# Eurus-Holmes/VAG-NMT

Hardware: AMD Instinct MI355X
Metric: training sentence-pairs/sec (Multi30K en->de, B=64) (higher is better)
Workload: dtype f32; 1 GPU; configs[1]: multimodal en->de train step, B=64/GPU, Ts=Tt=40, E=256, H=512, S=512, I=2048, Vs=8507, V=9391, dropout 0.3/0.5/0.5, tied emb, teacher_force_ratio=1; global_batch=64, parallelism=dp1, hip_graph=True

## Files before the change

### vag-nmt_amd/csrc/api.hip

```cpp
#include "../../include/vag_nmt.h"
#include "kernels.h"
#include <cstring>

#define S_(x) reinterpret_cast<hipStream_t>(x)

static inline int zero_async(void* p, size_t bytes, hipStream_t s) {
    if (bytes == 0) return VAG_OK;
    return vag_axpy_launch(0.f, reinterpret_cast<const float*>(p), reinterpret_cast<float*>(p), (int64_t)(bytes / 4), 2, s);
}
static inline int copy_async(void* dst, const void* src, size_t bytes, hipStream_t s) {
    if (bytes == 0) return VAG_OK;
    return vag_axpy_launch(1.f, reinterpret_cast<const float*>(src), reinterpret_cast<float*>(dst), (int64_t)(bytes / 4), 0, s);
}
static int linear_fwd(int64_t M, int64_t N, int64_t K, const float* x, int64_t ldx, const float* W, const float* bias,
                      int act, float* y, int64_t ldy, hipStream_t s) {
    if (M <= 256) return vag_skinny_launch(M, N, K, x, ldx, W, K, bias, nullptr, 0, y, ldy, act, s);
    return vag_gemm_launch(M, N, K, 1.f, x, ldx, 1, W, 1, K, 0.f, y, ldy, bias, act, s);
}
static int gemm_tn_acc(int64_t M, int64_t N, int64_t R, const float* A, int64_t lda, const float* B, int64_t ldb, float* C,
                       int64_t ldc, hipStream_t s, float* g_bias = nullptr) {
    if (R == 0) return VAG_OK;
    return vag_gemm_launch(M, N, R, 1.f, A, 1, lda, B, ldb, 1, 1.f, C, ldc, nullptr, VAG_ACT_NONE, s, 0, g_bias);
}
static int gemm_nn(int64_t M, int64_t N, int64_t K, const float* A, int64_t lda, const float* B, int64_t ldb, float beta,
// ... 31 lines not shown
}

static void* head_dl16_slot(float* logits, int64_t ldl, int64_t R, int64_t CH, int64_t E) {
    if (!head_grads_one_plane() || CH <= 128 || vag_opt().head_bf16_dlogits == 0) return nullptr;
    if (E <= 64 || vag_opt().gemm_f32mfma != 0 || vag_opt().gemm_force_tile != 0) return nullptr;
    if (CH * 3 > R * 2) return nullptr;
    return logits + CH * ldl;
}

VagOptions& vag_opt() {
    static VagOptions o;
    return o;
}

extern "C" {

int vag_version(void) { return 330; }

int vag_set_option(const char* name, int64_t value) {
    VAG_CHECK_ARG(name != nullptr);
    VagOptions& o = vag_opt();
    const struct { const char* n; int* p; } ints[] = {
        {"gemm_f32mfma", &o.gemm_f32mfma}, {"gemm_slabs", &o.gemm_slabs}, {"gemm_nogroup", &o.gemm_nogroup}, {"gemm_big", &o.gemm_big}, {"gemm_force_tile", &o.gemm_force_tile},
        {"gemm_force_splitk", &o.gemm_force_splitk}, {"head_fuse", &o.head_fuse},
        {"head_bf16_grads", &o.head_bf16_grads}, {"persistent", &o.persistent}, {"persistent_dec_bwd", &o.persistent_dec_bwd}, {"persistent_enc_bwd", &o.persistent_enc_bwd}, {"free_persistent", &o.free_persistent}, {"attn_dot_reg", &o.attn_dot_reg},
        {"persist_timing", &o.persist_timing}, {"s16_one_plane", &o.s16_one_plane}, {"leaf_queue", &o.leaf_queue}, {"attn_row", &o.attn_row}, {"dec_xcd_map", &o.dec_xcd_map}, {"loss_ride", &o.loss_ride}, {"step_fork", &o.step_fork},
        {"head_bf16_dlogits", &o.head_bf16_dlogits}};
    for (const auto& e : ints)
        if (strcmp(name, e.n) == 0) { *e.p = (int)value; return VAG_OK; }
    if (strcmp(name, "head_chunk") == 0) { o.head_chunk = value; return VAG_OK; }
    if (strcmp(name, "persist_spin_limit") == 0) { o.persist_spin_limit = value; return VAG_OK; }
#ifdef VAG_LAB
    if (strcmp(name, "dec_stamps") == 0) { o.dec_stamps = value; return VAG_OK; }
    if (strcmp(name, "dec_bwd_stamps") == 0) { o.dec_bwd_stamps = value; return VAG_OK; }
    if (strcmp(name, "gemm_debug") == 0) { o.gemm_debug = (int)value; return VAG_OK; }
    if (strcmp(name, "gemm_planes") == 0) {
        g_base_ctx.gemm_planes = (value == 2 || value == 1 || value == 11) ? (int)value : 3;
        return VAG_OK;
    }
#endif
    return VAG_EINVAL;
}

int vag_set_operator_context(const float* derived, int storage) {
    VAG_CHECK_ARG(storage == 0 || (storage == 1 && derived));
    g_base_ctx.derived = derived;
    g_base_ctx.store16 = storage == 1;
// ... 945 lines not shown
    const int64_t R = Tt * B;
    if (!inv_cnt_ready) VAG_TRY(vag_inv_cnt_launch(tgt, B, Tt, inv_cnt, s));
    VagCallCtx::HeadFuse& hf = vag_ctx().head_fuse;
    const int64_t hc = vag_ctx().head_chunk;
    const int64_t CH = (!logits_ready && hc > 0 && hc < R) ? (hc + B - 1) / B * B : 0;
    if (CH > 0) {
        VAG_TRY(head_pre_seq(h2_all, c_all, e_all, w, R, E, H, p_out, rng, tmid, s));
        for (int64_t r0 = 0; r0 < R; r0 += CH) {
            const int64_t rows = R - r0 < CH ? R - r0 : CH;
            VAG_TRY(vag_gemm_launch(rows, V, E, 1.f, tmid + r0 * E, E, 1, w.out_w, 1, E, 0.f, logits, ldl, w.out_b, 0, s));
            VAG_TRY(vag_lse_nll_launch(logits, ldl, rows, V, tgt + r0 / B, B, Tt, vocab_weight, lse + r0, nll + r0, nullptr, 0,
                                       nullptr, 0, s, eps));
            if (hf.g) {
                const vag_head_g& g = *hf.g;
                void* dl16 = rows > 128 ? head_dl16_slot(logits, ldl, R, CH, E) : nullptr;
                VAG_TRY(vag_ce_bwd_colsum_launch(logits, ldl, rows, V, tgt + r0 / B, B, Tt, vocab_weight, lse + r0, inv_cnt,
                                                 hf.d_loss, g.out_b, s, dl16, eps));
                VAG_TRY(head_dt_gemm(rows, E, V, logits, ldl, w.out_w, hf.dt + r0 * E, s, dl16));
                VAG_TRY(head_outw_gemm(V, E, rows, logits, ldl, tmid + r0 * E, g.out_w, s, dl16));
            }
        }
        if (hf.g) hf.done = true;
    } else {
        if (!logits_ready) {
            VAG_TRY(head_pre_seq(h2_all, c_all, e_all, w, R, E, H, p_out, rng, tmid, s));
            VAG_TRY(vag_gemm_launch(R, V, E, 1.f, tmid, E, 1, w.out_w, 1, E, 0.f, logits, ldl, w.out_b, 0, s));
        }
        VAG_TRY(vag_lse_nll_launch(logits, ldl, R, V, tgt, B, Tt, vocab_weight, lse, nll, nullptr, 0, nullptr, 0, s, eps));
    }
    if (losses) return vag_loss_mt_mix_launch(nll, inv_cnt, B, Tt, losses, w_mt, w_vse, has_vse, s);
    return vag_loss_mt_launch(nll, inv_cnt, B, Tt, loss_mt, s);
}
extern "C" {

static int head_bwd_data(const vag_head_w& w, int64_t R, int64_t E, int64_t H, int64_t V, float p_out, const uint64_t* rng,
                         const float* tmid, const float* dlogits, int64_t ldl, float* d_h2_all, float* d_c_all,
                         float* d_e_all, float* dt, hipStream_t s, bool dt_ready = false) {
    const int64_t C = 2 * H;
    if (!dt_ready) VAG_TRY(head_dt_gemm(R, E, V, dlogits, ldl, w.out_w, dt, s));
    VAG_TRY(vag_tanh_bwd_launch(tmid, dt, dt, R * E, rng, VAG_DROP_DEC_OUT, p_out, s));
    VagGemmGroup grp5;
    VAG_TRY(gemm_nn(R, H, E, dt, E, w.w1, H, 0.f, d_h2_all, H, s));
    VAG_TRY(gemm_nn(R, C, E, dt, E, w.w2, C, 0.f, d_c_all, C, s));
    VAG_TRY(gemm_nn(R, E, E, dt, E, w.w3, E, 0.f, d_e_all, E, s));
    return grp5.end(s);
}
static int head_bwd_weights(const float* h2_all, const float* c_all, const float* e_all, int64_t R, int64_t E, int64_t H,
                            int64_t V, const float* tmid, const float* dlogits, int64_t ldl, const float* dt,
                            const vag_head_g& g, hipStream_t s, bool out_b_done = false, bool out_w_done = false) {
    const int64_t C = 2 * H;
    VagGemmGroup grp6;
// ... 548 lines not shown
```

### vag-nmt_amd/csrc/call_ctx.h

```cpp
#pragma once
#include <hip/hip_runtime.h>
#include <stdint.h>
#include "../../include/vag_nmt.h"

struct LossTask {
    const float* nll = nullptr; const float* inv_cnt = nullptr; float* losses = nullptr;
    int B = 0, Tt = 0, has_vse = 0, ring = 0;
    float w_mt = 0.f, w_vse = 0.f;
};
struct RmwDefer {
    float* out = nullptr;
    const float *a1 = nullptr, *x1 = nullptr, *a2 = nullptr, *x2 = nullptr;
    const float *mask = nullptr, *dx = nullptr; float coef = 0.f;
    int64_t B = 0, Ts = 0, C = 0;
};

struct VagCallCtx {
    const float* derived = nullptr;
    bool store16 = false;
    int gemm_planes = 3;
    unsigned* guard = nullptr;

    int64_t head_chunk = 0;
    struct HeadFuse { const vag_head_g* g = nullptr; const float* d_loss = nullptr; float* dt = nullptr; bool done = false; } head_fuse;
    bool step_zeroed = false;
    bool step_gathered = false;
    bool poison_inject = false;
    bool persist_prezeroed = false;
    int loss_ring = 0;
    struct GemmScratch { float* slab = nullptr; int64_t floats = 0; unsigned* tickets = nullptr; int64_t ntickets = 0; hipStream_t stream = nullptr; } gemm_scratch;
    const float* gemm_prezeroed[4] = {nullptr, nullptr, nullptr, nullptr};
    struct LeafStream { hipStream_t stream = nullptr; hipEvent_t event = nullptr; bool used = false; } leaf_stream;

    struct RowMix { float* xmix = nullptr; float split = 0.f; const float* done = nullptr; } row_mix;
    struct Dh0Tanh { bool req = false; const float* done = nullptr; } dh0_tanh;
    struct LossDefer { bool on = false; LossTask task; hipStream_t stream = nullptr; } loss_defer;
    RmwDefer rmw;
    bool leaf_on = false;
    const float* u_all_ready = nullptr;
};

VagCallCtx& vag_ctx();

struct VagCallScope {
    VagCallCtx& ctx;
    VagCallCtx* prev;
    explicit VagCallScope(VagCallCtx& c);
    ~VagCallScope();
    VagCallScope(const VagCallScope&) = delete;
    VagCallScope& operator=(const VagCallScope&) = delete;
};
```

### vag-nmt_amd/csrc/common.h

```cpp
#pragma once
#include <hip/hip_runtime.h>
#include <stdint.h>
#include <stddef.h>

#define VAG_OK 0
#define VAG_EINVAL (-22)
#define VAG_ENOSYS (-38)

#define VAG_CHECK_ARG(cond)                     \
    do {                                        \
        if (!(cond)) return VAG_EINVAL;         \
    } while (0)

#define VAG_LAUNCH_CHECK()                                  \
    do {                                                    \
        hipError_t e__ = hipGetLastError();                 \
        if (e__ != hipSuccess) return (int)e__;             \
    } while (0)

#define VAG_TRY(expr)                  \
    do {                               \
        int r__ = (expr);              \
        if (r__ != 0) return r__;      \
    } while (0)
// ... 51 lines not shown
__device__ __forceinline__ float h16_hi(unsigned p) { return (float)__builtin_bit_cast(vag_half, (unsigned short)(p >> 16)); }
template <bool XH> __device__ __forceinline__ float4 ld4_any(const float* base, int64_t elem) {
    if (XH) {
        const uint2 p = *reinterpret_cast<const uint2*>(reinterpret_cast<const vag_half*>(base) + elem);
        return make_float4(h16_lo(p.x), h16_hi(p.x), h16_lo(p.y), h16_hi(p.y));
    }
    return *reinterpret_cast<const float4*>(base + elem);
}
template <bool XH> __device__ __forceinline__ float ld1_any(const float* base, int64_t elem) {
    if (XH) return (float)reinterpret_cast<const vag_half*>(base)[elem];
    return base[elem];
}

struct VagOptions {
    int gemm_f32mfma = 0;
    int gemm_big = 1;
    int gemm_slabs = 1;
    int gemm_nogroup = 0;
    int gemm_force_tile = 0;
    int gemm_force_splitk = 0;
    int gemm_debug = 0;
    int64_t head_chunk = -1;
    int head_fuse = 1;
    int head_bf16_grads = 1;
    int persistent = 1;
    int persistent_dec_bwd = 1;
    int persistent_enc_bwd = 1;
    int attn_dot_reg = 1;
    int free_persistent = 1;
    int s16_one_plane = 1;
    int head_bf16_dlogits = 1;
    int leaf_queue = 1;
    int attn_row = 1;
    int loss_ride = 1;
    int dec_xcd_map = 33;
    int step_fork = 0;
    int64_t persist_spin_limit = 0;
    int persist_timing = 0;
    int64_t dec_bwd_stamps = 0;
    int64_t dec_stamps = 0;
};
VagOptions& vag_opt();

enum { VAG_ACT_NONE = 0, VAG_ACT_TANH = 1 };
enum { VAG_DROP_ENC_EMB = 1, VAG_DROP_ENC_CTX = 2, VAG_DROP_DEC_OUT = 3 };

// ... 94 lines not shown
```

### vag-nmt_amd/csrc/gemm.hip

```cpp
#ifndef VAG_CHEAT_B
#define VAG_CHEAT_B 0
#endif
#include "gemm_shared.h"
#include "call_ctx.h"
#include <algorithm>
#include <atomic>
#include <cstdio>
#include <cstdlib>
#include <functional>
int vag_copy2d_launch(const float* in, int64_t ldi, float* out, int64_t ldo, int64_t rows, int64_t cols, hipStream_t s);

template <int BT, bool KC, bool VEC, int NTH>
__device__ __forceinline__ void tile_load(const float* __restrict__ P, int64_t so, int64_t sk, int o0, int k0,
                                          int OUT, int KEND, float4 (&r)[BT * (BK / 4) / NTH]) {
    const int tid = threadIdx.x;
#pragma unroll
    for (int i = 0; i < BT * (BK / 4) / NTH; ++i) {
        const int idx = tid + i * NTH;
        float4 v = make_float4(0.f, 0.f, 0.f, 0.f);
        if (KC) {
            const int o = o0 + idx / (BK / 4), k = k0 + ((idx % (BK / 4)) << 2);
            if (o < OUT) {
                const float* p = P + (int64_t)o * so + k;
                if (VEC && k + 3 < KEND) {
// ... 131 lines not shown
    int tiles_x[LEAF_MAX];
    int n;
};
__global__ __launch_bounds__(256) void gemm_tiled_multi_kernel(LeafTasks T) {
    __shared__ __attribute__((aligned(16))) float smem[2 * BK * 68 + 2 * BK * 68];
    int k = 0;
    while (k + 1 < T.n && (int)blockIdx.x >= T.tile0[k + 1]) ++k;
    const int t = blockIdx.x - T.tile0[k];
    const GemmArgs& a = T.g[k];
    const int bx = t % T.tiles_x[k], by = t / T.tiles_x[k];
    if (a.rowsum && bx == 0 && threadIdx.x < 64) {
        const int m = by * 64 + threadIdx.x;
        if (m < a.M) {
            float s0 = 0.f, s1 = 0.f;
            int r = 0;
            for (; r + 1 < a.K; r += 2) { s0 += a.A[(int64_t)r * a.sa_k + m]; s1 += a.A[(int64_t)(r + 1) * a.sa_k + m]; }
            if (r < a.K) s0 += a.A[(int64_t)r * a.sa_k + m];
            a.rowsum[m] += s0 + s1;
        }
    }
    gemm_tiled_body<64, 64, false, false, true, 256>(a, smem, bx, by, 0);
}

template <bool AKC, bool BKC, bool VEC, int PL = 3, bool F16 = false, bool ABF = false>
__device__ __forceinline__ void gemm_split_body(const GemmArgs& a, __bf16* smem, int bx, int by, int bz) {
    __bf16* As = smem;
    __bf16* Bs = smem + PL * SP_PLANE;
    const int m0 = by * 128, n0 = bx * 128;
    const int kbeg = bz * a.kchunk;
    const int kend = min(a.K, kbeg + a.kchunk);
    const int lane = threadIdx.x & 63, wave = threadIdx.x >> 6;
    const int wm = wave >> 2, wn = wave & 3;

    f32x16 acc[2];
#pragma unroll
    for (int i = 0; i < 2; ++i)
#pragma unroll
        for (int r = 0; r < 16; ++r) acc[i][r] = 0.f;

    const __bf16* Af = As + (wm * 64 + (lane & 31)) * SP_LD + 8 * (lane >> 5);
    const __bf16* Bf = Bs + (wn * 32 + (lane & 31)) * SP_LD + 8 * (lane >> 5);

    SpRegs ra, rb;
    constexpr bool FAST = VEC && !ABF;
    const int nt = (kend - kbeg + SP_BK - 1) / SP_BK;
    const int nfull = FAST ? (kend - kbeg) / SP_BK : 0;
    SpFast<AKC> fa;
// ... 75 lines not shown
            for (int r = 0; r < 16; ++r) acc[i][r] = 0.f;
        const float4* all = reinterpret_cast<const float4*>(a.slab) + (int64_t)tile * a.nslices * 4096 + (wave * 8) * 64 + lane;
        for (int z = 0; z < a.nslices; ++z) {
            f32x4 v[8];
            const float4* p = all + (int64_t)z * 4096;
            asm volatile("global_load_dwordx4 %0, %8, off sc1\n\tglobal_load_dwordx4 %1, %8, off offset:1024 sc1\n\t"
                         "global_load_dwordx4 %2, %8, off offset:2048 sc1\n\tglobal_load_dwordx4 %3, %8, off offset:3072 sc1\n\t"
                         "global_load_dwordx4 %4, %9, off sc1\n\tglobal_load_dwordx4 %5, %9, off offset:1024 sc1\n\t"
                         "global_load_dwordx4 %6, %9, off offset:2048 sc1\n\tglobal_load_dwordx4 %7, %9, off offset:3072 sc1\n\t"
                         "s_waitcnt vmcnt(0)"
                         : "=&v"(v[0]), "=&v"(v[1]), "=&v"(v[2]), "=&v"(v[3]), "=&v"(v[4]), "=&v"(v[5]), "=&v"(v[6]), "=&v"(v[7])
                         : "v"(p), "v"(p + 256) : "memory");
#pragma unroll
            for (int i = 0; i < 2; ++i)
#pragma unroll
                for (int q = 0; q < 4; ++q)
#pragma unroll
                    for (int e = 0; e < 4; ++e) acc[i][4 * q + e] += v[i * 4 + q][e];
        }
        atomic = a.beta != 0.f;
        first = true;
    }
    const int col = n0 + wn * 32 + (lane & 31);
    if (col >= a.N) return;
    const float bv = (a.bias && first) ? a.bias[col] : 0.f;
#pragma unroll
    for (int i = 0; i < 2; ++i) {
        const int row0 = m0 + wm * 64 + i * 32 + 4 * (lane >> 5);
        if (a.c_half) gemm_epilogue16(acc[i], a.C, a.ldc, a.M - row0, a.alpha, a.beta, bv, a.act, atomic, 1, (int64_t)row0 * a.ldc + col);
        else gemm_epilogue16(acc[i], a.C + (int64_t)row0 * a.ldc + col, a.ldc, a.M - row0, a.alpha, a.beta, bv, a.act, atomic);
    }
}

template <bool AKC, bool BKC, bool VEC, int PL = 3, bool F16 = false, bool ABF = false>
__global__ __launch_bounds__(512, PL == 1 ? 6 : 4) void gemm_split_kernel(GemmArgs a) {
    __shared__ __attribute__((aligned(16))) __bf16 smem[2 * PL * SP_PLANE];
    gemm_split_body<AKC, BKC, VEC, PL, F16, ABF>(a, smem, blockIdx.x, blockIdx.y, blockIdx.z);
}

template <bool AKC, bool BKC, int PL = 3, bool F16 = false>
__global__ __launch_bounds__(512, PL == 1 ? 6 : 4) void gemm_split_group_kernel(GemmGroupArgs G) {
    __shared__ __attribute__((aligned(16))) __bf16 smem[2 * PL * SP_PLANE];
    int p = 0;
    while (p + 1 < G.n && (int)blockIdx.x >= G.start[p + 1]) ++p;
    const GemmArgs& a = G.p[p];
    const int id = blockIdx.x - G.start[p];
    const int tn = (a.N + 127) / 128, tm = (a.M + 127) / 128;
    const int bx = id % tn, by = (id / tn) % tm, bz = id / (tn * tm);
    gemm_split_body<AKC, BKC, true, PL, F16>(a, smem, bx, by, bz);
}

constexpr int BIG_STAGE = 4 * SP_PLANE;
constexpr int BIG_LDS_BYTES = 2 * BIG_STAGE * 2;
__device__ __forceinline__ void big_barrier() { asm volatile("s_waitcnt lgkmcnt(0)\n\ts_barrier" ::: "memory"); }

template <bool AKC, bool BKC, bool F16, bool ABF>
__device__ __forceinline__ void gemm_big_body(const GemmArgs& a, __bf16* smem, int bx, int by, int bz) {
    const int m0 = by * 256, n0 = bx * 256;
    const int kbeg = bz * a.kchunk;
    const int kend = min(a.K, kbeg + a.kchunk);
// ... 138 lines not shown
    const GemmArgs& a = G.p[p];
    const int id = blockIdx.x - G.start[p];
    const int tn = (a.N + 255) / 256, tm = (a.M + 255) / 256;
    const int bx = id % tn, by = (id / tn) % tm, bz = id / (tn * tm);
    gemm_big_body<AKC, BKC, F16, false>(a, big_smem, bx, by, bz);
}
template <typename K> static bool big_attr(K kernel) {
    static std::atomic<unsigned long long> done{0};
    int dev = 0;
    if (hipGetDevice(&dev) != hipSuccess || dev < 0 || dev >= 64) return false;
    if (done.load(std::memory_order_acquire) & (1ull << dev)) return true;
    if (hipFuncSetAttribute(reinterpret_cast<const void*>(kernel), hipFuncAttributeMaxDynamicSharedMemorySize, BIG_LDS_BYTES) != hipSuccess)
        return false;
    done.fetch_or(1ull << dev, std::memory_order_release);
    return true;
}

static int gemm_split_dispatch(const GemmArgs& g, bool akc, bool bkc, bool vec, dim3 grid, hipStream_t s) {
    const int gemm_planes = vag_ctx().gemm_planes;
    if (g.a_bf16) {
        if (gemm_planes != 1 || bkc || !vec) return VAG_EINVAL;
        if (akc) hipLaunchKernelGGL((gemm_split_kernel<true, false, true, 1, false, true>), grid, dim3(512), 0, s, g);
        else hipLaunchKernelGGL((gemm_split_kernel<false, false, true, 1, false, true>), grid, dim3(512), 0, s, g);
        VAG_LAUNCH_CHECK();
        return VAG_OK;
    }
#define VAG_SPLIT_CASE(AK, BKc, V)                                                                    \
    if (akc == AK && bkc == BKc && vec == V) {                                                        \
        if (gemm_planes == 2) hipLaunchKernelGGL((gemm_split_kernel<AK, BKc, V, 2>), grid, dim3(512), 0, s, g);   \
        else if (gemm_planes == 1) hipLaunchKernelGGL((gemm_split_kernel<AK, BKc, V, 1>), grid, dim3(512), 0, s, g);   \
        else if (gemm_planes == 11) hipLaunchKernelGGL((gemm_split_kernel<AK, BKc, V, 1, true>), grid, dim3(512), 0, s, g);   \
        else hipLaunchKernelGGL((gemm_split_kernel<AK, BKc, V, 3>), grid, dim3(512), 0, s, g);        \
        VAG_LAUNCH_CHECK();                                                                           \
        return VAG_OK;                                                                                \
    }
    VAG_SPLIT_CASE(true, true, true)
    VAG_SPLIT_CASE(true, false, true)
    VAG_SPLIT_CASE(false, true, true)
    VAG_SPLIT_CASE(false, false, true)
    VAG_SPLIT_CASE(true, true, false)
    VAG_SPLIT_CASE(true, false, false)
    VAG_SPLIT_CASE(false, true, false)
    VAG_SPLIT_CASE(false, false, false)
#undef VAG_SPLIT_CASE
    return VAG_EINVAL;
}
// ... 347 lines not shown
            if (sp > 1 && (!can_split || K / sp < 128)) break;
            const int64_t kper = cdiv64(cdiv64(K, sp), BK) * BK;
            const int64_t blocks = base * sp;
            double rounds;
            if (t == 128 && !opt_f32mfma) {
                const int64_t full = blocks / 512, rem = blocks % 512;
                rounds = 1.5 * (double)full + (rem == 0 ? 0.0 : (rem <= 256 ? 1.0 : 1.5));
            } else {
                rounds = (double)cdiv64(blocks, 256);
            }
            const double t_mfma = rounds * (double)kper * (double)(t * t) * 2.0 / (256.0 * eff) / 2400.0;
            const double bytes = (double)M * (double)N * 4.0;
            const bool slabs_on = gemm_slabs_usable(stream) && t == 128 && gemm_planes == 3 && !opt_f32mfma;
            const double t_out = sp > 1 ? (slabs_on ? sp * bytes / 4.0e6 + 1.5 * sp + bytes / (beta != 0.f ? atomic_rate : 4.0e6)
                                                    : sp * bytes / atomic_rate + (beta == 0.f ? bytes / 4.0e6 + 2.0 : 0.0))
                                        : bytes * (beta != 0.f ? 2.0 : 1.0) / 4.0e6;
            const double cost = t_mfma + t_out;
            if (cost < best) { best = cost; T = t; splitk = sp; }
        }
    }
    {
        const int ft = vag_opt().gemm_force_tile, fs = vag_opt().gemm_force_splitk;
        if ((ft == 64 || ft == 128) && fs >= 1 && (fs == 1 || can_split)) { T = ft; splitk = fs; }
    }
#ifdef VAG_LAB
    if (vag_opt().gemm_debug)
        fprintf(stderr, "[vag_gemm] M=%lld N=%lld K=%lld akc=%d bkc=%d beta=%g -> T=%lld splitk=%lld model=%.1f us\n",
                (long long)M, (long long)N, (long long)K, (int)akc, (int)bkc, (double)beta, (long long)T, (long long)splitk, best);
#endif
    if (T == 128 && (gemm_planes == 1 || gemm_planes == 11) && vec && !opt_f32mfma && vag_opt().gemm_big != 0 && M >= 192 && N >= 192 &&
        (!a_bf16 || !bkc) && vag_opt().gemm_force_tile == 0) {
        const int64_t tiles = cdiv64(M, 256) * cdiv64(N, 256);
        int64_t sp = 1;
        if (can_split) while (tiles * sp < 208 && K / (sp + 1) >= 512 && sp < 32) ++sp;
        int kc = (int)(cdiv64(cdiv64(K, sp), BK) * BK);
        sp = cdiv64(K, kc);
        g.splitk = (int)sp; g.kchunk = kc;
        if (sp > 1 && beta == 0.f && !gemm_take_prezeroed(C)) {
            int64_t nb = cdiv64(M * N, 256 * 8);
            if (nb > 2048) nb = 2048;
            hipLaunchKernelGGL(fill2d_kernel, dim3((unsigned)nb), dim3(256), 0, stream, C, ldc, M, N);
            VAG_LAUNCH_CHECK();
        }
        const dim3 grid((unsigned)cdiv64(N, 256), (unsigned)cdiv64(M, 256), (unsigned)sp);
        const bool f16 = gemm_planes == 11;
#define VAG_BIG1(AK, BKc, F, AB)                                                                                              \
// ... 1301 lines not shown
```

### vag-nmt_amd/csrc/gemm_shared.h

```cpp
#pragma once
#include "common.h"

struct GemmArgs {
    const float* A; const float* B; float* C; const float* bias;
    int64_t sa_o, sa_k;
    int64_t sb_o, sb_k;
    int64_t ldc;
    int M, N, K, kchunk;
    float alpha, beta;
    int act, splitk;
    int c_half;
    int a_bf16;
    float* rowsum;
    float* slab;
    unsigned* ticket;
    int nslices;
};


constexpr int BK = 32;

__device__ __forceinline__ void gemm_epilogue16(const f32x16& acc, float* __restrict__ cbase, int64_t ldc, int rows_left,
                                                float alpha, float beta, float bv, int act, bool atomic, int c_half = 0,
                                                int64_t c_elem0 = 0) {
    if (rows_left <= 0) return;
    if (c_half) {
        vag_half* ch = reinterpret_cast<vag_half*>(cbase) + c_elem0;
#pragma unroll
        for (int r = 0; r < 16; ++r) {
            const int dr = (r & 3) + 8 * (r >> 2);
            float v = alpha * acc[r] + bv;
            if (act == VAG_ACT_TANH) v = vag_tanh(v);
            if (dr < rows_left) ch[(int64_t)dr * ldc] = (vag_half)v;
        }
        return;
    }
    if (atomic) {
#pragma unroll
        for (int r = 0; r < 16; ++r) {
// ... 337 lines not shown
```

### vag-nmt_amd/csrc/head.hip

```cpp
#include "kernels.h"

__device__ __forceinline__ float block_reduce_max(float v, float* sh) {
    v = wave_max(v);
    const int lane = threadIdx.x & 63, w = threadIdx.x >> 6;
    if (lane == 0) sh[w] = v;
    __syncthreads();
    float r = sh[0];
    for (int i = 1; i < (int)(blockDim.x >> 6); ++i) r = fmaxf(r, sh[i]);
    __syncthreads();
    return r;
}
__device__ __forceinline__ float block_reduce_sum(float v, float* sh) {
    v = wave_sum(v);
    const int lane = threadIdx.x & 63, w = threadIdx.x >> 6;
    if (lane == 0) sh[w] = v;
    __syncthreads();
    float r = 0.f;
    for (int i = 0; i < (int)(blockDim.x >> 6); ++i) r += sh[i];
    __syncthreads();
    return r;
}

template <int NV, bool LS>
__global__ __launch_bounds__(256) void lse_nll_kernel(const float* __restrict__ logits, int64_t ldl, int V,
// ... 99 lines not shown
    }
}

int vag_lse_nll_launch(const float* logits, int64_t ldl, int64_t rows, int64_t V, const int64_t* tgt, int64_t B,
                       int64_t Tt, const float* vw, float* lse, float* nll, int64_t* argmax, int64_t argmax_stride,
                       float* logp_out, int64_t ldlp, hipStream_t s, float eps) {
    VAG_CHECK_ARG(logits && rows >= 0 && V > 0 && ldl >= V);
    VAG_CHECK_ARG(!tgt || (vw && nll && B > 0 && Tt > 0));
    VAG_CHECK_ARG(vag_label_smoothing_ok(eps) && (eps == 0.f || tgt));
    if (rows == 0) return VAG_OK;
#define VAG_LSE_GO(NV, LS)                                                                                              \
    hipLaunchKernelGGL((lse_nll_kernel<NV, LS>), dim3((unsigned)rows), dim3(256), 0, s, logits, ldl, (int)V, tgt, (int)B, \
                       (int)Tt, vw, lse, nll, argmax, argmax_stride, logp_out, ldlp, eps)
    if (eps > 0.f) {
        if (V <= 256 * 8) VAG_LSE_GO(8, true);
        else if (V <= 256 * 40) VAG_LSE_GO(40, true);
        else VAG_LSE_GO(0, true);
    } else {
        if (V <= 256 * 8) VAG_LSE_GO(8, false);
        else if (V <= 256 * 40) VAG_LSE_GO(40, false);
        else VAG_LSE_GO(0, false);
    }
#undef VAG_LSE_GO
    VAG_LAUNCH_CHECK();
    return VAG_OK;
}

__global__ __launch_bounds__(256) void inv_cnt_kernel(const int64_t* __restrict__ tgt, int B, int Tt,
                                                      float* __restrict__ inv_cnt) {
    const int b = blockIdx.x * 256 + threadIdx.x;
    if (b >= B) return;
    int c = 0;
    for (int t = 0; t < Tt; ++t) c += tgt[(int64_t)b * Tt + t] != 0;
    inv_cnt[b] = 1.f / (float)c;
}
int vag_inv_cnt_launch(const int64_t* tgt, int64_t B, int64_t Tt, float* inv_cnt, hipStream_t s) {
    VAG_CHECK_ARG(tgt && inv_cnt && B > 0 && Tt > 0);
    hipLaunchKernelGGL(inv_cnt_kernel, dim3((unsigned)cdiv64(B, 256)), dim3(256), 0, s, tgt, (int)B, (int)Tt, inv_cnt);
    VAG_LAUNCH_CHECK();
    return VAG_OK;
}

__device__ __forceinline__ void loss_mt_body(float (&sh)[4], const float* __restrict__ nll, const float* __restrict__ inv_cnt,
                                             int B, int Tt, float* __restrict__ loss, float* __restrict__ losses,
                                             float w_mt, float w_vse, int has_vse, int ring) {
    const int g = threadIdx.x >> 6, lane = threadIdx.x & 63;
// ... 218 lines not shown
```

### vag-nmt_amd/csrc/kernels.h

```cpp
#pragma once
#include "common.h"
#include "call_ctx.h"
#include "../../include/vag_nmt.h"

int vag_embed_gather_launch(const int64_t* idx, int64_t ist, int64_t isb, int64_t T, int64_t B, const float* W,
                            int64_t E, float* out, const uint64_t* rng, int sid, float p, hipStream_t s,
                            float* mask_out = nullptr);
int vag_embed_scatter_launch(const int64_t* idx, int64_t ist, int64_t isb, int64_t T, int64_t B, const float* g,
                             int64_t E, float* gW, const uint64_t* rng, int sid, float p, hipStream_t s,
                             const unsigned* poison = nullptr);

struct GruBwdSide {
    const float* dh_carry;
    const float* dh_add;
    int64_t drop_idx0;
    const float* save;
    const float* hprev;
    float* dgi;
    float* dgh;
    float* dh_prev;
    int t;
};
struct GruBwdArgs {
    GruBwdSide s[2];
// ... 40 lines not shown
int vag_attn_ctx_gru_launch(const float* scores, const float* encwp, int64_t N, int64_t rps, int64_t Ts, int64_t H,
                            const float* b_ih, const float* hp, int64_t ldhp, const float* hprev, float* alpha, float* hout,
                            float* save, hipStream_t s, bool x16 = false,
                            const float* x2 = nullptr, int64_t W2 = 0, float* out2 = nullptr);
int vag_attn_wsum_launch(int over_src, const float* a, const float* x, int64_t B, int64_t Ts, int64_t T, int64_t W, float* out,
                         hipStream_t s);
int vag_attn_ctx_launch(int softmax, const float* scores, const float* enc, int64_t N, int64_t rps, int64_t Ts,
                        int64_t C, float* alpha, float* ctx, hipStream_t s);
int vag_softmax_bwd_launch(const float* alpha, const float* dalpha, int64_t N, int64_t Ts, float* dscore, hipStream_t s);
int vag_attn_dq_launch(const float* pe, const float* q, int64_t ldq, const float* v, const float* alpha,
                       const float* dalpha, float* dscore, int64_t N, int64_t Ts, int64_t C, float* dq, int64_t lddq,
                       hipStream_t s, bool x16 = false);
int vag_attn_post_bwd_launch(const float* pe, const float* q_all, int64_t ldq, const float* v, const float* ds_all,
                             const float* alpha_all, const float* dc_all, int64_t B, int64_t Ts, int64_t Tt,
                             int64_t C, float* d_pe, float* dvp, float* d_enc, int accumulate_enc, hipStream_t s,
                             bool x16 = false);
int vag_outer2_launch(const float* a1, const float* x1, const float* a2, const float* x2, int64_t B, int64_t Ts,
                      int64_t C, float* out, int accumulate, hipStream_t s);

inline bool vag_label_smoothing_ok(float eps) { return eps >= 0.f && eps < 1.f; }
int vag_lse_nll_launch(const float* logits, int64_t ldl, int64_t rows, int64_t V, const int64_t* tgt, int64_t B,
                       int64_t Tt, const float* vw, float* lse, float* nll, int64_t* argmax, int64_t argmax_stride,
                       float* logp_out, int64_t ldlp, hipStream_t s, float eps);
int vag_inv_cnt_launch(const int64_t* tgt, int64_t B, int64_t Tt, float* inv_cnt, hipStream_t s);
int vag_loss_mt_launch(const float* nll, const float* inv_cnt, int64_t B, int64_t Tt, float* loss, hipStream_t s);
int vag_loss_mt_mix_launch(const float* nll, const float* inv_cnt, int64_t B, int64_t Tt, float* losses, float w_mt,
                           float w_vse, int has_vse, hipStream_t s);
int vag_ce_bwd_launch(float* logits, int64_t ldl, int64_t rows, int64_t V, const int64_t* tgt, int64_t B, int64_t Tt,
                      const float* vw, const float* lse, const float* inv_cnt, const float* d_loss, hipStream_t s,
                      float eps);
int vag_ce_bwd_colsum_launch(float* logits, int64_t ldl, int64_t rows, int64_t V, const int64_t* tgt, int64_t B, int64_t Tt,
                             const float* vw, const float* lse, const float* inv_cnt, const float* d_loss, float* g_bias,
                             hipStream_t s, void* out16, float eps);

int vag_logsoftmax_bwd_launch(const float* logp, int64_t ldlp, float* d, int64_t ldd, int64_t rows, int64_t V,
                              hipStream_t s);

int vag_l2norm_fwd_launch(const float* y, int64_t B, int64_t S, float* nrm, float* out, hipStream_t s);
int vag_l2norm_bwd_launch(const float* y, const float* nrm, const float* out, const float* d_out, int64_t B, int64_t S,
                          int act, float* dy, hipStream_t s);
int vag_rank_loss_launch(const float* scores, int64_t B, float margin, int kind, float* G, float* loss, hipStream_t s,
                         const float* g_scale = nullptr);
int vag_retrieval_rank_launch(const float* scores, int64_t N, int* ranks, hipStream_t s);
int vag_scale_by_dev_launch(float* x, int64_t n, const float* scalar, hipStream_t s);

int vag_clip_adam_shard_launch(float* p, float* g, float* m, float* v, int64_t n, int nseg, const int64_t* seg_off,
// ... 130 lines not shown
```

### vag-nmt_amd/csrc/step.hip

```cpp
#include "../../include/vag_nmt.h"
#include <vector>
#include "kernels.h"

#define S_(x) reinterpret_cast<hipStream_t>(x)

namespace {

struct StepWs {
    float *enc, *mask, *ws_enc, *pe;
    float *y_im, *nrm_im, *im_emb, *ws_img, *alpha_v, *ctx, *y_txt, *nrm_txt, *txt_emb, *rscores, *G;
    float *xmix, *hseq, *c_all, *e_all, *ws_dec, *tmid, *logits, *lse, *nll, *inv_cnt, *consts;
    int64_t* tok;
    float *d_enc, *d_pe, *d_h2, *d_c, *d_e, *d_h0, *d_ctx, *d_im, *d_txt, *scr_dec, *scr_head, *scr_ini;
    float* free_tab;
    float* gemm_slab;
    unsigned* gemm_ticket;
    int64_t gemm_slab_floats, gemm_tickets;
    int64_t total;
};

StepWs step_ws(float* p, const vag_step_cfg& c) {
    StepWs w;
    const int64_t B = c.B, Ts = c.Ts, Tt = c.Tt, H = c.H, C = 2 * c.H, S = c.S, R = c.Tt * c.B;
    int64_t o = 0;
    auto take = [&](int64_t n) { float* q = p ? p + o : nullptr; o += (n + 63) & ~63ll; return q; };
    w.enc = take(B * Ts * C); w.mask = take(B * Ts); w.ws_enc = take(vag_bigru_ws_floats(B, Ts, c.Es, H));
    w.pe = take(B * Ts * C);
    const bool mm = c.multimodal != 0;
    w.y_im = take(mm ? B * S : 0); w.nrm_im = take(mm ? B : 0); w.im_emb = take(mm ? B * S : 0);
    w.ws_img = take(mm ? vag_imagine_ws_floats(B, Ts, C, S, c.attn_method) : 0);
    w.alpha_v = take(mm ? B * Ts : 0); w.ctx = take(mm ? B * C : 0);
    w.y_txt = take(mm ? B * S : 0); w.nrm_txt = take(mm ? B : 0); w.txt_emb = take(mm ? B * S : 0);
    w.rscores = take(mm ? B * B : 0); w.G = take(mm ? B * B : 0);
    w.xmix = take(B * C); w.hseq = take((Tt + 1) * B * H); w.c_all = take(R * C); w.e_all = take(R * c.Et);
    w.ws_dec = take(vag_cgru_ws_floats(B, Ts, Tt, c.Et, H));
    w.tmid = take(R * c.Et); w.logits = take(R * c.ldl); w.lse = take(R); w.nll = take(R); w.inv_cnt = take(B);
    w.consts = take(8);
    w.tok = reinterpret_cast<int64_t*>(take(2 * (Tt + 1) * B));
    w.d_enc = take(B * Ts * C); w.d_pe = take(B * Ts * C); w.d_h2 = take(R * H); w.d_c = take(R * C); w.d_e = take(R * c.Et);
    w.d_h0 = take(B * H); w.d_ctx = take(mm ? B * C : 0); w.d_im = take(mm ? B * S : 0); w.d_txt = take(mm ? B * S : 0);
    w.scr_dec = take(vag_cgru_bwd_scratch_floats(B, Ts, Tt, c.Et, H)); w.scr_head = take(R * c.Et); w.scr_ini = take(B * C);
    w.free_tab = take(H == 512 && c.Et == 256 && B <= 64 ? vag_dec_free_tables_floats(B, Ts, Tt, c.Et, H, c.V) : 0);
    const int64_t widest = std::max(std::max(B * Ts * C, R * 3 * H), std::max(3 * H * C, R * c.Et));
    w.gemm_slab_floats = c.storage == 0 ? std::min<int64_t>(12 * widest, 192ll << 20) : 0;
    w.gemm_tickets = c.storage == 0 ? 16384 : 0;
    w.gemm_slab = take(w.gemm_slab_floats);
    w.gemm_ticket = reinterpret_cast<unsigned*>(take(w.gemm_tickets));
    w.total = o;
    return w;
}

bool cfg_ok(const vag_step_cfg* c) {
    return c && c->B > 0 && c->Ts > 0 && c->Tt > 0 && c->Es > 0 && c->Et > 0 && c->H > 0 && c->V > 0 && c->Es % 4 == 0 &&
           c->Et % 4 == 0 && c->H % 4 == 0 && c->ldl >= c->V && c->ldl % 4 == 0 && c->loss_ring >= 0 && (reinterpret_cast<uintptr_t>(c->guard) & 3) == 0 &&
           vag_label_smoothing_ok(c->label_smoothing) &&
           (!c->multimodal || (c->S > 0 && c->S % 4 == 0 && c->I > 0 && (c->attn_method == 0 || c->attn_method == 1) &&
                               c->rank_kind >= -1 && c->rank_kind <= 1));
}

struct ZeroRanges { uint4* p[6]; int64_t n[6]; };
struct GatherTask { const float* emb; float* out; int E4; };
__global__ __launch_bounds__(256) void step_prologue_kernel(uint64_t* rng, const int64_t* __restrict__ tgt, int B, int Tt,
                                                            int64_t* __restrict__ tok, float* __restrict__ consts,
                                                            float* __restrict__ inv_cnt, float w_mt, float w_vse,
                                                            unsigned* __restrict__ z0, int64_t n0, unsigned* __restrict__ z1,
// ... 39 lines not shown

extern "C" {

int64_t vag_step_ws_floats(const vag_step_cfg* cfg) {
    if (!cfg_ok(cfg)) return VAG_EINVAL;
    return step_ws(nullptr, *cfg).total;
}

int64_t vag_step_ws_offset(const vag_step_cfg* cfg, int which) {
    if (!cfg_ok(cfg)) return VAG_EINVAL;
    static float base[1];
    StepWs w = step_ws(base, *cfg);
    const float* p = nullptr;
    switch (which) {
        case 0: p = w.enc; break;
        case 1: p = w.alpha_v; break;
        case 2: p = w.hseq; break;
        case 3: p = w.logits; break;
        case 4: p = w.ws_dec; break;
        case 5: p = w.d_enc; break;
        case 6: p = w.im_emb; break;
        case 7: p = w.txt_emb; break;
        case 8: p = reinterpret_cast<const float*>(w.tok); break;
        default: return VAG_EINVAL;
    }
    return (int64_t)(p - base);
}

}

namespace {
struct ForkState { hipStream_t side = nullptr; hipEvent_t ev[6] = {nullptr, nullptr, nullptr, nullptr, nullptr, nullptr}; int dev = -1; };
thread_local ForkState g_fork[8];
ForkState* fork_state() {
    int dev = 0;
    if (hipGetDevice(&dev) != hipSuccess) { (void)hipGetLastError(); return nullptr; }
    ForkState* f = nullptr;
    for (auto& x : g_fork) if (x.dev == dev) { f = &x; break; }
    if (!f) for (auto& x : g_fork) if (x.dev < 0) { f = &x; break; }
    if (!f) return nullptr;
    if (!f->side) {
        int lo = 0, hi = 0;
        if (hipDeviceGetStreamPriorityRange(&lo, &hi) != hipSuccess) { (void)hipGetLastError(); lo = 0; }
        if (hipStreamCreateWithPriority(&f->side, hipStreamNonBlocking, lo) != hipSuccess) { (void)hipGetLastError(); f->side = nullptr; return nullptr; }
        for (auto& e : f->ev)
            if (hipEventCreateWithFlags(&e, hipEventDisableTiming) != hipSuccess) { (void)hipGetLastError(); return nullptr; }
// ... 35 lines not shown
    const vag_step_cfg& c = *cfg;
    const vag_model_w& w = *wp;
    const vag_model_g& g = *gp;
    const bool mm = c.multimodal != 0;
    VAG_CHECK_ARG(!mm || (im && w.im_w && w.im_b && w.txt_w && w.txt_b && w.ctx2ctx && w.emb2ctx &&
                          (c.attn_method == 0 || w.mlp_w)));
    VAG_CHECK_ARG(w.enc_emb && w.ini_w && w.ini_b && w.attn_e && (phases & 55) != 0 && (phases & ~55) == 0);
    const int64_t B = c.B, Ts = c.Ts, Tt = c.Tt, H = c.H, C = 2 * H, S = c.S, V = c.V, Et = c.Et;
    StepWs k = step_ws(ws, c);
    VAG_CHECK_ARG(c.storage == 0 || (c.storage == 1 && derived && !c.free_run && H % 8 == 0));
    int64_t chunk = 0;
    if (!c.free_run && (double)c.Tt * (double)c.B * (double)c.ldl * 4.0 > 1073741824.0) {
        chunk = (int64_t)(671088640.0 / ((double)c.ldl * 4.0)) / c.B * c.B;
        if (chunk < c.B) chunk = c.B;
    }
    if (vag_opt().head_chunk >= 0)
        chunk = c.free_run ? 0 : vag_opt().head_chunk;
    VagCallCtx ctx = vag_ctx();
    ctx.derived = derived;
    ctx.store16 = c.storage == 1;
    ctx.gemm_planes = ctx.store16 ? 2 : 3;
    ctx.head_chunk = chunk;
    ctx.loss_ring = c.loss_ring;
    if (c.guard) ctx.guard = reinterpret_cast<unsigned*>(c.guard);
    ctx.persist_prezeroed = true;
    ctx.step_zeroed = true;
    VagCallScope scope(ctx);
    const VagCallCtx::GemmScratch slabs = {k.gemm_slab, k.gemm_slab_floats, k.gemm_ticket, k.gemm_tickets, s};
    if (!(phases & 1)) ctx.gemm_scratch = slabs;
    if (chunk > 0 && (phases & 1) && (phases & (2 | 16)) && vag_opt().head_fuse != 0) {
        ctx.head_fuse.g = &g.head; ctx.head_fuse.d_loss = k.consts + 0; ctx.head_fuse.dt = k.scr_head;
    }
    const bool has_vse = mm && c.rank_kind >= 0;
    const float w_mt = mm ? c.loss_w : 1.f, w_vse = mm ? 1.f - c.loss_w : 0.f;
    float* h0 = k.hseq;
    float* h2_all = k.hseq + B * H;
    const uint64_t* crng = rng;
    float* d_e = vag_cgru_bwd_scratch_de(k.scr_dec, B, Ts, Tt, Et, H);
    const bool one_plane = c.storage == 1 && !c.free_run && vag_opt().s16_one_plane != 0;
    StepBranch br_im, br_leaf, br_dw;
    if (phases & 1) {
        if (one_plane) ctx.gemm_planes = 11;
        if (mm) {
            hipStream_t si = br_im.fork(s, 0, 1);
            VAG_TRY(vag_img_proj_l2_fwd(im, w.im_w, w.im_b, B, c.I, S, c.activation_vse, k.y_im, k.nrm_im, k.im_emb, si));
        }
// ... 124 lines not shown
```

Before: 21560 sentence-pairs/s.

## Fuse per-tile row max/sum-exp stats into head logits GEMM epilogue

Adds a STAT variant of the split GEMM kernel. When it computes the vocabulary logits, it also writes per-row, per-128-column-tile partial max, sum-exp and optional sum-x into a new workspace. A small finalize kernel then merges these partials into LSE and NLL, reading only the target logit. This replaces the full lse_nll pass that re-read the whole R×V logits matrix. The cost is extra shared-memory staging and syncs in the GEMM epilogue, and the logits GEMM is forced to T=128 with no split-K.

```diff
diff --git a/vag-nmt_amd/csrc/api.hip b/vag-nmt_amd/csrc/api.hip
--- a/vag-nmt_amd/csrc/api.hip
+++ b/vag-nmt_amd/csrc/api.hip
@@ -77,7 +77,7 @@
     VagOptions& o = vag_opt();
     const struct { const char* n; int* p; } ints[] = {
         {"gemm_f32mfma", &o.gemm_f32mfma}, {"gemm_slabs", &o.gemm_slabs}, {"gemm_nogroup", &o.gemm_nogroup}, {"gemm_big", &o.gemm_big}, {"gemm_force_tile", &o.gemm_force_tile},
-        {"gemm_force_splitk", &o.gemm_force_splitk}, {"head_fuse", &o.head_fuse},
+        {"gemm_force_splitk", &o.gemm_force_splitk}, {"head_fuse", &o.head_fuse}, {"head_ce_fused", &o.head_ce_fused},
         {"head_bf16_grads", &o.head_bf16_grads}, {"persistent", &o.persistent}, {"persistent_dec_bwd", &o.persistent_dec_bwd}, {"persistent_enc_bwd", &o.persistent_enc_bwd}, {"free_persistent", &o.free_persistent}, {"attn_dot_reg", &o.attn_dot_reg},
         {"persist_timing", &o.persist_timing}, {"s16_one_plane", &o.s16_one_plane}, {"leaf_queue", &o.leaf_queue}, {"attn_row", &o.attn_row}, {"dec_xcd_map", &o.dec_xcd_map}, {"loss_ride", &o.loss_ride}, {"step_fork", &o.step_fork},
         {"head_bf16_dlogits", &o.head_bf16_dlogits}};
@@ -1069,11 +1069,23 @@
         }
         if (hf.g) hf.done = true;
     } else {
+        bool stat_done = false;
         if (!logits_ready) {
             VAG_TRY(head_pre_seq(h2_all, c_all, e_all, w, R, E, H, p_out, rng, tmid, s));
-            VAG_TRY(vag_gemm_launch(R, V, E, 1.f, tmid, E, 1, w.out_w, 1, E, 0.f, logits, ldl, w.out_b, 0, s));
+            VagCallCtx::RowStat& rq = vag_ctx().row_stat;
+            if (rq.ws && vag_opt().head_ce_fused != 0 && !vag_ctx().store16) {
+                rq.part = rq.ws; rq.floats = rq.ws_floats; rq.ls = eps > 0.f; rq.done = nullptr;
+            }
+            const int rc = vag_gemm_launch(R, V, E, 1.f, tmid, E, 1, w.out_w, 1, E, 0.f, logits, ldl, w.out_b, 0, s);
+            rq.part = nullptr;
+            VAG_TRY(rc);
+            stat_done = rq.ws != nullptr && rq.done == rq.ws;
+            rq.done = nullptr;
         }
-        VAG_TRY(vag_lse_nll_launch(logits, ldl, R, V, tgt, B, Tt, vocab_weight, lse, nll, nullptr, 0, nullptr, 0, s, eps));
+        if (stat_done)
+            VAG_TRY(vag_head_stat_final_launch(vag_ctx().row_stat.ws, logits, ldl, R, V, tgt, B, Tt, vocab_weight, lse, nll, s, eps));
+        else
+            VAG_TRY(vag_lse_nll_launch(logits, ldl, R, V, tgt, B, Tt, vocab_weight, lse, nll, nullptr, 0, nullptr, 0, s, eps));
     }
     if (losses) return vag_loss_mt_mix_launch(nll, inv_cnt, B, Tt, losses, w_mt, w_vse, has_vse, s);
     return vag_loss_mt_launch(nll, inv_cnt, B, Tt, loss_mt, s);
diff --git a/vag-nmt_amd/csrc/call_ctx.h b/vag-nmt_amd/csrc/call_ctx.h
--- a/vag-nmt_amd/csrc/call_ctx.h
+++ b/vag-nmt_amd/csrc/call_ctx.h
@@ -34,6 +34,8 @@
 
     struct RowMix { float* xmix = nullptr; float split = 0.f; const float* done = nullptr; } row_mix;
     struct Dh0Tanh { bool req = false; const float* done = nullptr; } dh0_tanh;
+    struct RowStat { float* part = nullptr; bool ls = false; int64_t floats = 0; const float* done = nullptr;
+                     float* ws = nullptr; int64_t ws_floats = 0; } row_stat;
     struct LossDefer { bool on = false; LossTask task; hipStream_t stream = nullptr; } loss_defer;
     RmwDefer rmw;
     bool leaf_on = false;
diff --git a/vag-nmt_amd/csrc/common.h b/vag-nmt_amd/csrc/common.h
--- a/vag-nmt_amd/csrc/common.h
+++ b/vag-nmt_amd/csrc/common.h
@@ -97,6 +97,7 @@
     int gemm_debug = 0;
     int64_t head_chunk = -1;
     int head_fuse = 1;
+    int head_ce_fused = 1;
     int head_bf16_grads = 1;
     int persistent = 1;
     int persistent_dec_bwd = 1;
diff --git a/vag-nmt_amd/csrc/gemm.hip b/vag-nmt_amd/csrc/gemm.hip
--- a/vag-nmt_amd/csrc/gemm.hip
+++ b/vag-nmt_amd/csrc/gemm.hip
@@ -177,7 +177,7 @@
     gemm_tiled_body<64, 64, false, false, true, 256>(a, smem, bx, by, 0);
 }
 
-template <bool AKC, bool BKC, bool VEC, int PL = 3, bool F16 = false, bool ABF = false>
+template <bool AKC, bool BKC, bool VEC, int PL = 3, bool F16 = false, bool ABF = false, bool STAT = false>
 __device__ __forceinline__ void gemm_split_body(const GemmArgs& a, __bf16* smem, int bx, int by, int bz) {
     __bf16* As = smem;
     __bf16* Bs = smem + PL * SP_PLANE;
@@ -299,6 +299,54 @@
         first = true;
     }
     const int col = n0 + wn * 32 + (lane & 31);
+    if (STAT) {
+        const float bv = (col < a.N && a.bias) ? a.bias[col] : 0.f;
+        constexpr int LDT = 132;
+        float* T = reinterpret_cast<float*>(smem);
+        const int ntile = (a.N + 127) >> 7, ns = a.rowstat_ls ? 3 : 2;
+        const int rl = threadIdx.x >> 3, seg = threadIdx.x & 7;
+#pragma unroll
+        for (int i = 0; i < 2; ++i) {
+            const int row0 = m0 + wm * 64 + i * 32 + 4 * (lane >> 5);
+            if (col < a.N) {
+                gemm_epilogue16(acc[i], a.C + (int64_t)row0 * a.ldc + col, a.ldc, a.M - row0, a.alpha, 0.f, bv, VAG_ACT_NONE, false);
+#pragma unroll
+                for (int r = 0; r < 16; ++r)
+                    T[(wm * 32 + 4 * (lane >> 5) + (r & 3) + 8 * (r >> 2)) * LDT + wn * 32 + (lane & 31)] = a.alpha * acc[i][r] + bv;
+            }
+            __syncthreads();
+            const float* tr = T + rl * LDT + seg * 16;
+            const int c0 = n0 + seg * 16;
+            float x[16];
+#pragma unroll
+            for (int q = 0; q < 4; ++q) {
+                const float4 v = *reinterpret_cast<const float4*>(tr + 4 * q);
+                x[4 * q + 0] = v.x; x[4 * q + 1] = v.y; x[4 * q + 2] = v.z; x[4 * q + 3] = v.w;
+            }
+            float mx = -INFINITY;
+#pragma unroll
+            for (int q = 0; q < 16; ++q) mx = fmaxf(mx, c0 + q < a.N ? x[q] : -INFINITY);
+            mx = fmaxf(mx, __shfl_xor(mx, 1, 64));
+            mx = fmaxf(mx, __shfl_xor(mx, 2, 64));
+            mx = fmaxf(mx, __shfl_xor(mx, 4, 64));
+            float se = 0.f, sx = 0.f;
+#pragma unroll
+            for (int q = 0; q < 16; ++q) {
+                se += c0 + q < a.N ? __expf(x[q] - mx) : 0.f;
+                sx += c0 + q < a.N ? x[q] : 0.f;
+            }
+            se += __shfl_xor(se, 1, 64); se += __shfl_xor(se, 2, 64); se += __shfl_xor(se, 4, 64);
+            if (a.rowstat_ls) { sx += __shfl_xor(sx, 1, 64); sx += __shfl_xor(sx, 2, 64); sx += __shfl_xor(sx, 4, 64); }
+            const int row = m0 + (rl >> 5) * 64 + i * 32 + (rl & 31);
+            if (seg == 0 && row < a.M) {
+                float* o = a.rowstat + ((int64_t)row * ntile + bx) * ns;
+                o[0] = mx; o[1] = se;
+                if (a.rowstat_ls) o[2] = sx;
+            }
+            __syncthreads();
+        }
+        return;
+    }
     if (col >= a.N) return;
     const float bv = (a.bias && first) ? a.bias[col] : 0.f;
 #pragma unroll
@@ -309,10 +357,10 @@
     }
 }
 
-template <bool AKC, bool BKC, bool VEC, int PL = 3, bool F16 = false, bool ABF = false>
+template <bool AKC, bool BKC, bool VEC, int PL = 3, bool F16 = false, bool ABF = false, bool STAT = false>
 __global__ __launch_bounds__(512, PL == 1 ? 6 : 4) void gemm_split_kernel(GemmArgs a) {
     __shared__ __attribute__((aligned(16))) __bf16 smem[2 * PL * SP_PLANE];
-    gemm_split_body<AKC, BKC, VEC, PL, F16, ABF>(a, smem, blockIdx.x, blockIdx.y, blockIdx.z);
+    gemm_split_body<AKC, BKC, VEC, PL, F16, ABF, STAT>(a, smem, blockIdx.x, blockIdx.y, blockIdx.z);
 }
 
 template <bool AKC, bool BKC, int PL = 3, bool F16 = false>
@@ -497,6 +545,12 @@
         if (gemm_planes != 1 || bkc || !vec) return VAG_EINVAL;
         if (akc) hipLaunchKernelGGL((gemm_split_kernel<true, false, true, 1, false, true>), grid, dim3(512), 0, s, g);
         else hipLaunchKernelGGL((gemm_split_kernel<false, false, true, 1, false, true>), grid, dim3(512), 0, s, g);
+        VAG_LAUNCH_CHECK();
+        return VAG_OK;
+    }
+    if (g.rowstat) {
+        if (gemm_planes != 3 || !akc || !bkc || !vec || grid.z != 1) return VAG_EINVAL;
+        hipLaunchKernelGGL((gemm_split_kernel<true, true, true, 3, false, false, true>), grid, dim3(512), 0, s, g);
         VAG_LAUNCH_CHECK();
         return VAG_OK;
     }
@@ -890,6 +944,16 @@
     {
         const int ft = vag_opt().gemm_force_tile, fs = vag_opt().gemm_force_splitk;
         if ((ft == 64 || ft == 128) && fs >= 1 && (fs == 1 || can_split)) { T = ft; splitk = fs; }
+    }
+    {
+        VagCallCtx::RowStat& rq = vag_ctx().row_stat;
+        if (rq.part) {
+            const bool ok = gemm_planes == 3 && akc && bkc && vec && alpha == 1.f && beta == 0.f && act == VAG_ACT_NONE && !c_half &&
+                            !a_bf16 && !rowsum && !opt_f32mfma && N > 64 && (int64_t)M * cdiv64(N, 128) * 3 <= rq.floats;
+            if (ok && K <= 256 && vag_opt().gemm_force_tile == 0) { T = 128; splitk = 1; }
+            if (ok && T == 128 && splitk == 1) { g.rowstat = rq.part; g.rowstat_ls = rq.ls ? 1 : 0; rq.done = rq.part; }
+            rq.part = nullptr;
+        }
     }
 #ifdef VAG_LAB
     if (vag_opt().gemm_debug)
diff --git a/vag-nmt_amd/csrc/gemm_shared.h b/vag-nmt_amd/csrc/gemm_shared.h
--- a/vag-nmt_amd/csrc/gemm_shared.h
+++ b/vag-nmt_amd/csrc/gemm_shared.h
@@ -15,6 +15,8 @@
     float* slab;
     unsigned* ticket;
     int nslices;
+    float* rowstat = nullptr;
+    int rowstat_ls = 0;
 };
 
 
diff --git a/vag-nmt_amd/csrc/head.hip b/vag-nmt_amd/csrc/head.hip
--- a/vag-nmt_amd/csrc/head.hip
+++ b/vag-nmt_amd/csrc/head.hip
@@ -145,6 +145,54 @@
         else VAG_LSE_GO(0, false);
     }
 #undef VAG_LSE_GO
+    VAG_LAUNCH_CHECK();
+    return VAG_OK;
+}
+
+template <bool LS>
+__global__ __launch_bounds__(256) void head_stat_final_kernel(const float* __restrict__ part, int NT,
+                                                              const float* __restrict__ logits, int64_t ldl, int V,
+                                                              const int64_t* __restrict__ tgt, int B, int Tt,
+                                                              const float* __restrict__ vw, float* __restrict__ lse,
+                                                              float* __restrict__ nll, int rows, float eps) {
+    constexpr int NS = LS ? 3 : 2;
+    const int lane = threadIdx.x & 63;
+    const int row = blockIdx.x * 4 + (threadIdx.x >> 6);
+    if (row >= rows) return;
+    const float* p = part + (int64_t)row * NT * NS;
+    float mx = -INFINITY, sum = 0.f, sx = 0.f;
+    for (int t = lane; t < NT; t += 64) {
+        const float tm = p[t * NS], ts = p[t * NS + 1];
+        if (tm > mx) { sum = sum * __expf(mx - tm) + ts; mx = tm; }
+        else sum += ts * __expf(tm - mx);
+        if (LS) sx += p[t * NS + 2];
+    }
+    const float bm = wave_max(mx);
+    sum = wave_sum(mx > -INFINITY ? sum * __expf(mx - bm) : 0.f);
+    if (LS) sx = wave_sum(sx);
+    if (lane == 0) {
+        const float l = bm + __logf(sum);
+        lse[row] = l;
+        const int t = row / B, b = row - t * B;
+        const int64_t tg = tgt[(int64_t)b * Tt + t];
+        const float xt = logits[(int64_t)row * ldl + tg];
+        if (LS) nll[row] = vw[tg] * (l - (1.f - eps) * xt - eps * (sx / (float)V));
+        else nll[row] = -vw[tg] * (xt - l);
+    }
+}
+int vag_head_stat_final_launch(const float* part, const float* logits, int64_t ldl, int64_t rows, int64_t V, const int64_t* tgt,
+                               int64_t B, int64_t Tt, const float* vw, float* lse, float* nll, hipStream_t s, float eps) {
+    VAG_CHECK_ARG(part && logits && tgt && vw && lse && nll && rows == B * Tt && V > 0 && ldl >= V && rows < (1ll << 30));
+    VAG_CHECK_ARG(vag_label_smoothing_ok(eps));
+    if (rows == 0) return VAG_OK;
+    const int NT = (int)cdiv64(V, 128);
+    const dim3 grid((unsigned)cdiv64(rows, 4));
+    if (eps > 0.f)
+        hipLaunchKernelGGL(head_stat_final_kernel<true>, grid, dim3(256), 0, s, part, NT, logits, ldl, (int)V, tgt, (int)B, (int)Tt, vw,
+                           lse, nll, (int)rows, eps);
+    else
+        hipLaunchKernelGGL(head_stat_final_kernel<false>, grid, dim3(256), 0, s, part, NT, logits, ldl, (int)V, tgt, (int)B, (int)Tt, vw,
+                           lse, nll, (int)rows, eps);
     VAG_LAUNCH_CHECK();
     return VAG_OK;
 }
diff --git a/vag-nmt_amd/csrc/kernels.h b/vag-nmt_amd/csrc/kernels.h
--- a/vag-nmt_amd/csrc/kernels.h
+++ b/vag-nmt_amd/csrc/kernels.h
@@ -86,6 +86,8 @@
 int vag_lse_nll_launch(const float* logits, int64_t ldl, int64_t rows, int64_t V, const int64_t* tgt, int64_t B,
                        int64_t Tt, const float* vw, float* lse, float* nll, int64_t* argmax, int64_t argmax_stride,
                        float* logp_out, int64_t ldlp, hipStream_t s, float eps);
+int vag_head_stat_final_launch(const float* part, const float* logits, int64_t ldl, int64_t rows, int64_t V, const int64_t* tgt,
+                               int64_t B, int64_t Tt, const float* vw, float* lse, float* nll, hipStream_t s, float eps);
 int vag_inv_cnt_launch(const int64_t* tgt, int64_t B, int64_t Tt, float* inv_cnt, hipStream_t s);
 int vag_loss_mt_launch(const float* nll, const float* inv_cnt, int64_t B, int64_t Tt, float* loss, hipStream_t s);
 int vag_loss_mt_mix_launch(const float* nll, const float* inv_cnt, int64_t B, int64_t Tt, float* losses, float w_mt,
diff --git a/vag-nmt_amd/csrc/step.hip b/vag-nmt_amd/csrc/step.hip
--- a/vag-nmt_amd/csrc/step.hip
+++ b/vag-nmt_amd/csrc/step.hip
@@ -16,6 +16,8 @@
     float* gemm_slab;
     unsigned* gemm_ticket;
     int64_t gemm_slab_floats, gemm_tickets;
+    float* head_part;
+    int64_t head_part_floats;
     int64_t total;
 };
 
@@ -41,6 +43,8 @@
     w.d_h0 = take(B * H); w.d_ctx = take(mm ? B * C : 0); w.d_im = take(mm ? B * S : 0); w.d_txt = take(mm ? B * S : 0);
     w.scr_dec = take(vag_cgru_bwd_scratch_floats(B, Ts, Tt, c.Et, H)); w.scr_head = take(R * c.Et); w.scr_ini = take(B * C);
     w.free_tab = take(H == 512 && c.Et == 256 && B <= 64 ? vag_dec_free_tables_floats(B, Ts, Tt, c.Et, H, c.V) : 0);
+    w.head_part_floats = c.storage == 0 && !c.free_run ? R * ((c.V + 127) / 128) * 3 : 0;
+    w.head_part = take(w.head_part_floats);
     const int64_t widest = std::max(std::max(B * Ts * C, R * 3 * H), std::max(3 * H * C, R * c.Et));
     w.gemm_slab_floats = c.storage == 0 ? std::min<int64_t>(12 * widest, 192ll << 20) : 0;
     w.gemm_tickets = c.storage == 0 ? 16384 : 0;
@@ -126,6 +130,9 @@
         case 6: p = w.im_emb; break;
         case 7: p = w.txt_emb; break;
         case 8: p = reinterpret_cast<const float*>(w.tok); break;
+        case 9: p = w.lse; break;
+        case 10: p = w.nll; break;
+        case 11: if (w.head_part_floats == 0) return VAG_EINVAL; p = w.head_part; break;
         default: return VAG_EINVAL;
     }
     return (int64_t)(p - base);
@@ -207,6 +214,7 @@
     ctx.gemm_planes = ctx.store16 ? 2 : 3;
     ctx.head_chunk = chunk;
     ctx.loss_ring = c.loss_ring;
+    if (chunk == 0 && k.head_part_floats > 0) { ctx.row_stat.ws = k.head_part; ctx.row_stat.ws_floats = k.head_part_floats; }
     if (c.guard) ctx.guard = reinterpret_cast<unsigned*>(c.guard);
     ctx.persist_prezeroed = true;
     ctx.step_zeroed = true;
```

Result: no change. 21580 sentence-pairs/s, median of 2 (+0.1%).
